# SuwoongHeo/neurecon

Hardware: AMD Instinct MI355X
Metric: rays/sec (4096 rays x 128 samples, 8-layer x256 SDF MLP) (higher is better)
Workload: dtype f16x3

## Files before the change

include/neurecon_hip.h:

```cpp
#ifndef NEURECON_HIP_H
#define NEURECON_HIP_H

#include <stddef.h>
#include <stdint.h>

#ifdef __cplusplus
extern "C" {
#endif

#define NR_OK 0
#define NR_ERR_ARG (-1)
#define NR_ERR_UNSUPPORTED (-2)
#define NR_ERR_HIP (-3)
#define NR_ERR_WORKSPACE (-4)

#define NR_PREC_FP32 0
#define NR_PREC_F16X3 1

#define NR_UPSAMPLE_OFFICIAL 0
#define NR_UPSAMPLE_DIRECT_USE 1
#define NR_UPSAMPLE_DIRECT_MORE 2

int nr_version(void);
const char* nr_last_error(void);
// ... 86 lines not shown
  float fixed_s;
  int N_nograd_samples;
  const float* t_nograd;
  void* workspace;
  size_t workspace_bytes;
  const float* u_rand;
  const float* t_out_rand;
  const float* s_dev;
  int sample_only;
  float* d_all_out;
  int no_mid_skip;
  int no_defer;
  int64_t max_chunk_rays;
  size_t max_workspace_bytes;
  const void* fold_packed;
} NrNeusArgs;

#define NR_DEFAULT_WORKSPACE_BYTES ((size_t)4 << 30)
#define NR_MIN_CHUNK_RAYS 4096

size_t nr_neus_workspace_bytes(const NrNeusArgs* a);
int nr_neus_render(const NrNeusArgs* a, void* stream);

size_t nr_neus_fold_packed_bytes(const NrSdfDesc* sdf, const NrRadDesc* rad);
int nr_neus_fold_pack(const NrSdfDesc* sdf, const NrRadDesc* rad, const float* W8, const float* b8, const float* W0,
                      const float* b0, void* packed, void* stream);
int nr_neus_fold_forward(const NrSdfDesc* sdf, const void* sdf_packed, const NrRadDesc* rad, const void* rad_packed,
                         const void* fold_packed, const float* pts, const float* vdir, int64_t vdir_div,
                         const float* normals, int64_t P, float* u, float* sdf_out, float* rgb, void* stream);

// ... 365 lines not shown
```

neurecon_amd/_lib.py:

```python
import ctypes
import os
import threading

import torch

HERE = os.path.dirname(os.path.abspath(__file__))
LIB_PATH = os.environ.get('NR_LIB', os.path.join(HERE, 'libnrhip.so'))

PREC_FP32 = 0
PREC_F16X3 = 1
UPSAMPLE = {'official_solution': 0, 'direct_use': 1, 'direct_more': 2}

_c_p = ctypes.c_void_p
_c_i = ctypes.c_int
_c_i64 = ctypes.c_int64
_c_f = ctypes.c_float
_c_d = ctypes.c_double
_c_sz = ctypes.c_size_t


class NrSdfDesc(ctypes.Structure):
    _fields_ = [('D', _c_i), ('W', _c_i), ('skip', _c_i), ('multires', _c_i), ('W_geo_feat', _c_i),
                ('precision', _c_i), ('siren', _c_i)]

# ... 14 lines not shown
        ('sdf', ctypes.POINTER(NrSdfDesc)), ('sdf_packed', _c_p),
        ('rad', ctypes.POINTER(NrRadDesc)), ('rad_packed', _c_p),
        ('s', _c_f), ('obj_bounding_radius', _c_f), ('near_bypass', _c_f), ('far_bypass', _c_f),
        ('N_samples', _c_i), ('N_importance', _c_i), ('N_upsample_iters', _c_i), ('calc_normal', _c_i),
        ('white_bkgd', _c_i),
        ('t_coarse', _c_p), ('u_fine', _c_p),
        ('rgb', _c_p), ('depth', _c_p), ('acc', _c_p), ('normals', _c_p),
        ('d_final', _c_p), ('sdf_out', _c_p), ('nablas_out', _c_p), ('radiance_out', _c_p),
        ('alpha_out', _c_p), ('cdf_out', _c_p), ('weights_out', _c_p),
        ('nerf', ctypes.POINTER(NrNerfDesc)), ('nerf_packed', _c_p), ('N_outside', _c_i), ('t_outside', _c_p),
        ('sigma_out', _c_p), ('radiance_bg_out', _c_p),
        ('upsample_algo', _c_i), ('fixed_s', _c_f), ('N_nograd_samples', _c_i), ('t_nograd', _c_p),
        ('workspace', _c_p), ('workspace_bytes', _c_sz),
        ('u_rand', _c_p), ('t_out_rand', _c_p), ('s_dev', _c_p), ('sample_only', _c_i), ('d_all_out', _c_p),
        ('no_mid_skip', _c_i), ('no_defer', _c_i), ('max_chunk_rays', _c_i64), ('max_workspace_bytes', _c_sz),
        ('fold_packed', _c_p),
    ]


class NrVolsdfArgs(ctypes.Structure):
    _fields_ = [
        ('rays_o', _c_p), ('rays_d', _c_p), ('n_rays', _c_i64),
        ('sdf', ctypes.POINTER(NrSdfDesc)), ('sdf_packed', _c_p),
        ('rad', ctypes.POINTER(NrRadDesc)), ('rad_packed', _c_p),
        ('alpha_net', _c_f), ('beta_net', _c_f), ('beta_plus_init', _c_f), ('eps', _c_f),
        ('near', _c_f), ('far', _c_f), ('obj_bounding_radius', _c_f), ('use_sphere_bg', _c_i),
        ('N_samples', _c_i), ('N_importance', _c_i), ('max_upsample_steps', _c_i), ('max_bisection_steps', _c_i),
        ('calc_normal', _c_i), ('white_bkgd', _c_i),
        ('t_coarse', _c_p), ('t_init', _c_p), ('u_up', _c_p), ('u_fine', _c_p),
        ('rgb', _c_p), ('depth', _c_p), ('acc', _c_p), ('normals', _c_p),
        ('d_vals', _c_p), ('sdf_out', _c_p), ('nablas_out', _c_p), ('radiance_out', _c_p),
# ... 287 lines not shown
```

neurecon_amd/csrc/nr_capi.hip:

```cpp
#include <algorithm>
#include <cmath>
#include <cstring>
#include <string>

#include "nr_common.h"
#include <cstdlib>
#include "nr_mlp.h"
#include "nr_tgemm.h"
#include "nr_neus.h"
#include "nr_volsdf.h"
#include "nr_unisurf.h"

namespace nr {

static thread_local std::string g_err;
void set_error(const std::string& msg) { g_err = msg; }

static size_t align256(size_t x) { return (x + 255) & ~(size_t)255; }
static int64_t chunk_bytes_host(int KB) { return (int64_t)(2 * KB + 1) * 1024; }

int check_sdf_desc(const NrSdfDesc* d) {
  NR_REQUIRE(d, NR_ERR_ARG, "null NrSdfDesc");
  if (d->siren) {
    NR_REQUIRE(d->D == 5 && d->W == 256 && d->skip < 0 && d->multires < 0 && d->W_geo_feat == 256,
// ... 183 lines not shown
  c.pts_nog = F(pl.o_ptsn); c.s_nog = F(pl.o_sn);
  const bool fused = !direct && !a.sample_only;
  c.nraw = fused ? c.nab_f : nullptr;
  c.idv = fused ? (int*)(ws + pl.o_idv) : nullptr;
  if (fused) {
    c.sdf_f = c.sv;
    c.nab_f = F(pl.o_nsort);
  }
  const bool defer = fused && neus_deferred(a, R);
  if (defer) {
    c.slabs = (float4*)(ws + pl.o_slabs);
    c.tflag = (int*)(ws + pl.o_tflag);
    c.tiles = (int*)(ws + pl.o_tiles);
    c.tcnt = (int*)(ws + pl.o_tcnt);
  }
  void* mlp_ws = ws + pl.o_mlp;
  const size_t mlp_bytes = a.workspace_bytes - pl.o_mlp;
  const SdfLayout SL = sdf_layout(*a.sdf);
  const RadLayout RL = rad_layout(*a.rad);
  auto sample_sdf = [&](const float* pts, int64_t P, float* sdf_out, int64_t slot0) -> int {
    if (defer)
      return launch_sdf_deferred(SL, a.sdf_packed, pts, P, sdf_out, nullptr, a.sdf->multires,
                                 (float4*)((char*)c.slabs + (size_t)(slot0 / 16) * kSlabColBytes), nullptr, nullptr,
                                 1, st);
    return launch_sdf(SL, a.sdf_packed, pts, P, sdf_out, fused ? c.nraw + slot0 * 3 : nullptr, nullptr,
                      a.sdf->multires, fused ? mlp_ws : nullptr, fused ? mlp_bytes : 0, st);
  };
  const dim3 blk(64), grd((R + 63) / 64);
  int rc;

  {
  ProfScope prof("neus_prologue", (double)R, st);
  hipLaunchKernelGGL(neus_prologue, grd, blk, 0, st, c, a.rays_o + ray0 * 3, a.rays_d + ray0 * 3, a.t_coarse,
                     a.obj_bounding_radius, a.near_bypass, a.far_bypass);
  }
  NR_HIP_CHECK(hipGetLastError());
  if (a.upsample_algo != NR_UPSAMPLE_DIRECT_MORE && (rc = sample_sdf(c.pts, (int64_t)a.N_samples * R, c.sv, 0)))
    return rc;
  if (a.upsample_algo == NR_UPSAMPLE_DIRECT_MORE) {
    hipLaunchKernelGGL(neus_nograd_points, grd, blk, 0, st, c);
    NR_HIP_CHECK(hipGetLastError());
    if ((rc = launch_sdf(SL, a.sdf_packed, c.pts_nog, (int64_t)c.n_nog * R, c.s_nog, nullptr, nullptr,
                         a.sdf->multires, nullptr, 0, st)))
      return rc;
  }
  if (direct) {
    ProfScope prof("neus_upsample", (double)R, st);
    const float* u = a.u_rand ? a.u_rand + ray0 * a.N_importance : a.u_fine;
    hipLaunchKernelGGL(neus_direct_upsample, grd, blk, 0, st, c, (int)(a.upsample_algo == NR_UPSAMPLE_DIRECT_MORE), u,
                       (int64_t)(a.u_rand ? a.N_importance : 0));
  }
  NR_HIP_CHECK(hipGetLastError());
  float* dvb[2] = {c.dv, F(pl.o_dv2)};
  float* svb[2] = {c.sv, F(pl.o_sv2)};
  int* idb[2] = {c.idv, fused ? (int*)(ws + pl.o_idv2) : nullptr};
  int cur = 0;
  auto merge = [&](int L) -> int {
    ProfScope prof("neus_merge", (double)R, st);
    const int64_t nt = (int64_t)(L + n_up) * R;
    hipLaunchKernelGGL(neus_merge, dim3((unsigned)((nt + 255) / 256)), dim3(256), 0, st, c, L, dvb[cur ^ 1],
                       svb[cur ^ 1], idb[cur ^ 1]);
    cur ^= 1;
    c.dv = dvb[cur];
    c.sv = svb[cur];
    c.idv = idb[cur];
    if (fused) c.sdf_f = c.sv;
    NR_HIP_CHECK(hipGetLastError());
    return NR_OK;
  };
  for (int it = 0; it < c.n_iters; ++it) {
    if (it > 0 && (rc = merge(a.N_samples + (it - 1) * n_up))) return rc;
    const int64_t slot0 = (int64_t)(a.N_samples + it * n_up) * R;
    NeusChunk cu = c;
    if (defer) cu.pts = c.pts + slot0 * 3;
    {
      ProfScope prof("neus_upsample", (double)R, st);
      const float* u = a.u_rand ? a.u_rand + ((int64_t)it * a.n_rays + ray0) * n_up : a.u_fine;
      const size_t lds1 = (5 * (size_t)c.S + 1) * sizeof(float);
      if (4 * lds1 <= 65536)
        hipLaunchKernelGGL((neus_upsample<4>), dim3((unsigned)((R + 3) / 4)), dim3(64), 4 * lds1, st, cu, it, u,
                           (int64_t)(a.u_rand ? n_up : 0));
      else
        hipLaunchKernelGGL((neus_upsample<1>), dim3((unsigned)R), dim3(64), lds1, st, cu, it, u,
                           (int64_t)(a.u_rand ? n_up : 0));
    }
    NR_HIP_CHECK(hipGetLastError());
    if ((rc = sample_sdf(cu.pts, (int64_t)n_up * R, c.snew, slot0))) return rc;
  }
  if (c.n_iters > 0 && (rc = merge(c.S - n_up))) return rc;
  if (defer) {
    const int64_t nslot = (int64_t)c.S * R;
    c.tshift = 0;
    NR_HIP_CHECK(hipMemsetAsync(c.nraw, 0, (size_t)nslot * 3 * sizeof(float), st));
    if (a.calc_normal && a.N_outside == 0) {
      NR_HIP_CHECK(hipMemsetAsync(c.tflag, 0, (size_t)nslot * sizeof(int), st));
      NR_HIP_CHECK(hipMemsetAsync(c.tcnt, 0, sizeof(int), st));
      const int64_t nq = (int64_t)(c.S - 1) * R;
      hipLaunchKernelGGL(neus_sample_need, dim3((unsigned)((nq + 255) / 256)), dim3(256), 0, st, c, a.s_dev, a.s);
      NR_HIP_CHECK(hipGetLastError());
      hipLaunchKernelGGL(neus_point_list, dim3((unsigned)((nslot + 1023) / 1024)), dim3(1024), 0, st, c, nslot);
      NR_HIP_CHECK(hipGetLastError());
      if ((rc = launch_sdf_deferred(SL, a.sdf_packed, c.pts, nslot, nullptr, c.nraw, a.sdf->multires, c.slabs, c.tiles,
                                    c.tcnt, 4, st)))
        return rc;
    }
  }
  if (a.sample_only) {
    hipLaunchKernelGGL(neus_write_dall, dim3((unsigned)(((int64_t)c.S * R + 255) / 256)), dim3(256), 0, st, c.dv,
                       (int64_t)R, c.S, ray0, a.d_all_out);
    NR_HIP_CHECK(hipGetLastError());
    return NR_OK;
  }
  {
    ProfScope prof("neus_points", (double)R, st);
    hipLaunchKernelGGL(neus_expand, dim3((unsigned)(((int64_t)c.S * R + 255) / 256)), dim3(256), 0, st, c,
                       (int)!(defer && a.N_outside > 0));
  }
  NR_HIP_CHECK(hipGetLastError());
  if (!fused && (rc = launch_sdf(SL, a.sdf_packed, c.pts, (int64_t)c.S * R, c.sdf_f, c.nab_f, nullptr,
                                 a.sdf->multires, mlp_ws, mlp_bytes, st)))
    return rc;
  const int64_t Pm = (int64_t)(c.S - 1) * R;
  const char* f8p = nullptr;
  const char* r0p = nullptr;
  if (a.fold_packed) {
    const FoldLayout FL = fold_layout(RL);
    f8p = (const char*)a.fold_packed + FL.f8_off;
    r0p = (const char*)a.fold_packed + FL.r0_off;
  }
  if (a.radiance_out || a.no_mid_skip) {
    if ((rc = launch_sdf(SL, a.sdf_packed, c.mids, Pm, c.sdf_m, c.nab_m, c.feat_m, a.sdf->multires, mlp_ws, mlp_bytes,
                         st, nullptr, 0, f8p)))
      return rc;
    if ((rc = launch_radiance(RL, a.rad_packed, c.mids, c.rd, 1, R, c.nab_m, c.feat_m, Pm, c.rad_m,
                              a.rad->multires_view, st, nullptr, r0p)))
      return rc;
  } else {
    char* wsb = (char*)a.workspace;
    int* cnt = (int*)(wsb + pl.o_mcnt);
    int* slot = (int*)(wsb + pl.o_mslot);
    float* midc = (float*)(wsb + pl.o_midc);
    float* vdc = (float*)(wsb + pl.o_mvd);
    float* radc = (float*)(wsb + pl.o_mrad);
    NR_HIP_CHECK(hipMemsetAsync(cnt, 0, sizeof(int), st));
    const dim3 g1((unsigned)((Pm + 255) / 256));
    hipLaunchKernelGGL(neus_mid_compact, dim3((unsigned)((Pm + 1023) / 1024)), dim3(1024), 0, st, c, a.s_dev, a.s, cnt,
                       slot, midc, vdc);
    NR_HIP_CHECK(hipGetLastError());
    if ((rc = launch_sdf(SL, a.sdf_packed, midc, Pm, c.sdf_m, c.nab_m, c.feat_m, a.sdf->multires, mlp_ws, mlp_bytes,
                         st, cnt, 1, f8p)))
      return rc;
    if ((rc = launch_radiance(RL, a.rad_packed, midc, vdc, 1, INT64_MAX, c.nab_m, c.feat_m, Pm, radc,
                              a.rad->multires_view, st, cnt, r0p)))
      return rc;
    hipLaunchKernelGGL(neus_mid_scatter, g1, dim3(256), 0, st, slot, radc, Pm, c.rad_m);
    NR_HIP_CHECK(hipGetLastError());
  }
  NeusOut o{ray0, a.rgb, a.depth, a.acc, a.normals, a.d_final, a.sdf_out, a.nablas_out,
            a.radiance_out, a.alpha_out, a.cdf_out, a.weights_out, a.sigma_out, a.radiance_bg_out};
  if (a.N_outside > 0) {
    hipLaunchKernelGGL(neus_outside_points, grd, blk, 0, st, c,
                       a.t_out_rand ? a.t_out_rand + ray0 * a.N_outside : (const float*)nullptr);
    NR_HIP_CHECK(hipGetLastError());
    const int64_t Po = (int64_t)(c.S - 1 + a.N_outside) * R;
    if (a.sigma_out || a.radiance_bg_out) {
      if ((rc = launch_nerf(nerf_layout(*a.nerf), a.nerf_packed, c.x4, c.rd, 1, R, Po, c.sig_o, c.rad_o, st)))
        return rc;
    } else {
      char* wsb = (char*)a.workspace;
      int* cnt = (int*)(wsb + pl.o_cnt);
      int* slot = (int*)(wsb + pl.o_slot);
// ... 4 lines not shown
      NR_HIP_CHECK(hipMemsetAsync(cnt, 0, sizeof(int), st));
      const dim3 g1((unsigned)((Po + 255) / 256));
      hipLaunchKernelGGL(neus_outside_compact, dim3((unsigned)((Po + 1023) / 1024)), dim3(1024), 0, st, c, cnt, slot,
                         x4c, vdc);
      NR_HIP_CHECK(hipGetLastError());
      if ((rc = launch_nerf(nerf_layout(*a.nerf), a.nerf_packed, x4c, vdc, 1, INT64_MAX, Po, sigc, radc, st, cnt)))
        return rc;
      hipLaunchKernelGGL(neus_outside_scatter, g1, dim3(256), 0, st, slot, sigc, radc, Po, c.sig_o, c.rad_o);
      NR_HIP_CHECK(hipGetLastError());
    }
    if (defer) {
      const int64_t nslot = (int64_t)c.S * R;
      c.tshift = 0;
      if (a.calc_normal) {
        NR_HIP_CHECK(hipMemsetAsync(c.tflag, 0, (size_t)nslot * sizeof(int), st));
        NR_HIP_CHECK(hipMemsetAsync(c.tcnt, 0, sizeof(int), st));
        hipLaunchKernelGGL(neus_sample_need_outside, dim3((unsigned)((nslot + 255) / 256)), dim3(256), 0, st, c,
                           a.s_dev, a.s);
        NR_HIP_CHECK(hipGetLastError());
        hipLaunchKernelGGL(neus_point_list, dim3((unsigned)((nslot + 1023) / 1024)), dim3(1024), 0, st, c, nslot);
        NR_HIP_CHECK(hipGetLastError());
        if ((rc = launch_sdf_deferred(SL, a.sdf_packed, c.pts, nslot, nullptr, c.nraw, a.sdf->multires, c.slabs,
                                      c.tiles, c.tcnt, 4, st)))
          return rc;
      }
      hipLaunchKernelGGL(neus_gather_nablas, dim3((unsigned)((nslot + 255) / 256)), dim3(256), 0, st, c);
      NR_HIP_CHECK(hipGetLastError());
    }
    ProfScope prof("neus_composite", (double)R, st);
    const int M = c.S - 1 + a.N_outside;
    const size_t lds1 = (6 * (size_t)M + 4 * (size_t)c.S) * sizeof(float);
// ... 904 lines not shown
```

neurecon_amd/csrc/nr_neus.h:

```cpp
#pragma once
#include "nr_common.h"

namespace nr {

constexpr int kMaxUp = 32;

struct NeusChunk {
  int R;
  int N_samples;
  int n_up;
  int n_iters;
  int S;
  float* ro; float* rd; float* near; float* far;
  float* dv; float* sv; float* wtmp; float* dnew; float* snew;
  float* pts; float* mids; float* dmid;
  float* sdf_f; float* nab_f;
  float* nraw; int* idv;
  float4* slabs; int* tflag; int* tiles; int* tcnt; int tshift;
  float* sdf_m; float* nab_m; float* feat_m; float* rad_m;
  int N_out;
  float r_obj;
  const float* t_out;
  float* d_out; float* x4; float* sig_o; float* rad_o;
  int n_imp;
  int n_nog;
  float fixed_s;
  const float* t_nog;
  float* pts_nog; float* s_nog;
};

struct NeusOut {
  int64_t ray0;
  float* rgb; float* depth; float* acc; float* normals;
// ... 10 lines not shown
  size_t o_mslot, o_midc, o_mvd, o_mrad, o_mcnt;
  size_t o_slabs, o_tflag, o_tiles, o_tcnt;
  size_t total;
};

NeusPlan neus_plan(const NrNeusArgs& a, int64_t Rc);
bool neus_deferred(const NrNeusArgs& a, int64_t R);
int neus_total_samples(const NrNeusArgs& a);
__global__ void neus_sample_need(NeusChunk c, const float* s_dev, float s_val);
__global__ void neus_tile_list(NeusChunk c, int64_t n_tiles);
__global__ void neus_point_list(NeusChunk c, int64_t n_slots);
__global__ void neus_sample_need_outside(NeusChunk c, const float* s_dev, float s_val);
__global__ void neus_gather_nablas(NeusChunk c);

__global__ void neus_prologue(NeusChunk c, const float* rays_o, const float* rays_d, const float* t_coarse,
                              float r_obj, float near_bypass, float far_bypass);
template <int RPW>
__global__ void neus_upsample(NeusChunk c, int it, const float* u, int64_t u_stride);
__global__ void neus_merge(NeusChunk c, int L, float* dv2, float* sv2, int* idv2);
__global__ void neus_expand(NeusChunk c, int gather);
template <int RPW>
__global__ void neus_composite(NeusChunk c, NeusOut o, const float* s_dev, float s_val, int calc_normal, int white_bkgd);
__global__ void neus_outside_points(NeusChunk c, const float* t_rand);
__global__ void neus_outside_compact(NeusChunk c, int* count, int* slot, float* x4c, float* vdc);
__global__ void neus_mid_compact(NeusChunk c, const float* s_dev, float s_val, int* count, int* slot, float* midc,
                                 float* vdc);
__global__ void neus_mid_scatter(const int* slot, const float* radc, int64_t n, float* rad_m);
__global__ void neus_outside_scatter(const int* slot, const float* sigc, const float* radc, int64_t n, float* sig_o,
                                     float* rad_o);
__global__ void neus_nograd_points(NeusChunk c);
__global__ void neus_direct_upsample(NeusChunk c, int more, const float* u, int64_t u_stride);
__global__ void neus_composite_outside(NeusChunk c, NeusOut o, const float* s_dev, float s_val, int calc_normal,
                                       int white_bkgd);
// ... 9 lines not shown
```

neurecon_amd/csrc/nr_neus.hip:

```cpp
#include "nr_common.h"
#include "nr_mlp.h"
#include "nr_neus.h"

namespace nr {

__device__ __forceinline__ float4 load3(const float* p) { return make_float4(p[0], p[1], p[2], 0.f); }

__device__ __forceinline__ void normalize3(float& x, float& y, float& z) {
  const float n = norm3_ref(x, y, z);
  const float d = fmaxf(n, 1e-12f);
  x = fdiv(x, d);
  y = fdiv(y, d);
  z = fdiv(z, d);
}

__global__ __launch_bounds__(64) void neus_prologue(NeusChunk c, const float* __restrict__ rays_o, const float* __restrict__ rays_d,
                              const float* __restrict__ t_coarse, float r_obj, float near_bypass, float far_bypass) {
  const int r = blockIdx.x * blockDim.x + threadIdx.x;
  if (r >= c.R) return;
  const float ox = rays_o[r * 3 + 0], oy = rays_o[r * 3 + 1], oz = rays_o[r * 3 + 2];
  float dx = rays_d[r * 3 + 0], dy = rays_d[r * 3 + 1], dz = rays_d[r * 3 + 2];
  normalize3(dx, dy, dz);
  c.ro[r * 3 + 0] = ox; c.ro[r * 3 + 1] = oy; c.ro[r * 3 + 2] = oz;
  c.rd[r * 3 + 0] = dx; c.rd[r * 3 + 1] = dy; c.rd[r * 3 + 2] = dz;
  const float mid = -fadd(fadd(fmul(ox, dx), fmul(oy, dy)), fmul(oz, dz));
  float nr = fmaxf(fsub(mid, r_obj), 0.0f);
  float fr = fmaxf(fadd(mid, r_obj), r_obj);
  if (!__builtin_isnan(near_bypass)) nr = near_bypass;
  if (!__builtin_isnan(far_bypass)) fr = far_bypass;
  c.near[r] = nr;
  c.far[r] = fr;
  for (int s = 0; s < c.N_samples; ++s) {
    const float t = t_coarse[s];
// ... 41 lines not shown
    w[i * stride] = (float)acc;
  }
  auto cdf = [&](int j) { return j == 0 ? 0.0f : w[(int64_t)(j - 1) * stride]; };
  for (int k = 0; k < n; ++k) {
    const float uk = u[k];
    int lo = 0, hi = L;
    while (lo < hi) {
      const int m = (lo + hi) >> 1;
      if (cdf(m) >= uk) hi = m; else lo = m + 1;
    }
    const int below = lo > 0 ? lo - 1 : 0, above = lo < L - 1 ? lo : L - 1;
    out[k * out_stride] = invert_one(uk, cdf(below), cdf(above), bins[below * stride], bins[above * stride]);
  }
}

template <int RPW>
__global__ __launch_bounds__(64) void neus_upsample(NeusChunk c, int it, const float* __restrict__ u, int64_t u_stride) {
  extern __shared__ float lds[];
  constexpr int NL = 64 / RPW;
  const int r = blockIdx.x * RPW + (int)threadIdx.x / NL, l = (int)threadIdx.x % NL;
  const int L = c.N_samples + it * c.n_up;
  const int64_t R = c.R;
  const bool live = r < R;
  const int Ll = live ? L : 0;
  float* sz = lds + ((int)threadIdx.x / NL) * (5 * c.S + 1);
  float* ss = sz + c.S;
  float* sa = ss + c.S;
  float* scdf = sa + c.S;
  float* sq = scdf + c.S;
  float* stot = sq + c.S;
  for (int i = l; i < Ll; i += NL) {
    sz[i] = c.dv[i * R + r];
    ss[i] = c.sv[i * R + r];
  }
  __syncthreads();
  const float S = (float)(64 << it);
  for (int i = l; i < Ll - 1; i += NL) {
    const float s0 = ss[i], s1 = ss[i + 1], z0 = sz[i], z1 = sz[i + 1];
    const float mid = fmul(fadd(s0, s1), 0.5f);
    const float slope = fdiv(fsub(s1, s0), fadd(fsub(z1, z0), 1e-5f));
    const float prev_slope = i > 0 ? fdiv(fsub(s0, ss[i - 1]), fadd(fsub(z0, sz[i - 1]), 1e-5f)) : 0.0f;
    float m = fminf(prev_slope, slope);
    m = fminf(fmaxf(m, -10.0f), 0.0f);
    const float dist = fsub(z1, z0);
    const float md = fmul(fmul(m, dist), 0.5f);
    const float c0 = sigmoidf_ref(fmul(fsub(mid, md), S));
    const float c1 = sigmoidf_ref(fmul(fadd(mid, md), S));
    const float alpha = fdiv(fadd(fsub(c0, c1), 1e-5f), fadd(c0, 1e-5f));
    sa[i] = alpha;
    scdf[i] = fadd(fsub(1.0f, alpha), 1e-10f);
// ... 33 lines not shown
    } else {
      int lo = 0, hi = L - 1;
      while (lo < hi) {
        const int mm = (lo + hi) >> 1;
        if (uk <= scdf[mm + 1]) hi = mm; else lo = mm + 1;
      }
      d = lo < L - 1 ? invert_one(uk, scdf[lo], scdf[lo + 1], sz[lo], sz[lo + 1])
                     : invert_one(uk, scdf[L - 1], scdf[L - 1], sz[L - 1], sz[L - 1]);
    }
    const int64_t q = k * R + r;
    c.dnew[q] = d;
    c.pts[q * 3 + 0] = fadd(ox, fmul(dx, d));
    c.pts[q * 3 + 1] = fadd(oy, fmul(dy, d));
    c.pts[q * 3 + 2] = fadd(oz, fmul(dz, d));
  }
}

template __global__ void neus_upsample<1>(NeusChunk, int, const float*, int64_t);
template __global__ void neus_upsample<4>(NeusChunk, int, const float*, int64_t);

__device__ __forceinline__ float merge_key(float v) { return v != v ? __builtin_inff() : v; }

__global__ void neus_merge(NeusChunk c, int L, float* __restrict__ dv2, float* __restrict__ sv2,
                           int* __restrict__ idv2) {
  const int64_t R = c.R;
  const int n = c.n_up;
  const int64_t t = (int64_t)blockIdx.x * blockDim.x + threadIdx.x;
  if (t >= (int64_t)(L + n) * R) return;
  const int64_t e = t / R, r = t - e * R;
  if (e < L) {
    const int64_t q = e * R + r;
    const float d = c.dv[q], kd = merge_key(d);
    int cnt = 0;
    for (int k = 0; k < n; ++k) cnt += merge_key(c.dnew[k * R + r]) < kd ? 1 : 0;
    const int64_t qo = (e + cnt) * R + r;
    dv2[qo] = d;
// ... 76 lines not shown
  float* snrm = srad + 3 * S;
  float* sdm = snrm + 3 * S;
  for (int i = l; i < Sl; i += NL) {
    const float cdf = sigmoidf_ref(fmul(c.sdf_f[i * R + r], s_inv));
    scdf[i] = cdf;
    if (o.cdf) o.cdf[ro * S + i] = cdf;
  }
  __syncthreads();
  for (int i = l; i < Sl - 1; i += NL) {
    const float cp = scdf[i], cn = scdf[i + 1];
    const float alpha = fmaxf(fdiv(fsub(cp, cn), fadd(cp, 1e-10f)), 0.0f);
    sal[i] = alpha;
    if (o.alpha) o.alpha[ro * (S - 1) + i] = alpha;
    const int64_t q = i * R + r;
    sdm[i] = c.dmid[q];
#pragma unroll
    for (int e = 0; e < 3; ++e) srad[i * 3 + e] = c.rad_m[q * 3 + e];
    if (calc_normal) {
      float x = c.nab_f[q * 3 + 0], y = c.nab_f[q * 3 + 1], z = c.nab_f[q * 3 + 2];
      normalize3(x, y, z);
      snrm[i * 3 + 0] = x;
      snrm[i * 3 + 1] = y;
      snrm[i * 3 + 2] = z;
    }
  }
  __syncthreads();
  double rgb0 = 0.0, rgb1 = 0.0, rgb2 = 0.0, n0 = 0.0, n1 = 0.0, n2 = 0.0;
  float accf = 0.0f;
  if (l == 0 && live) {
    double T = 1.0, acc = 0.0;
    for (int i = 0; i < S - 1; ++i) {
      const float alpha = sal[i];
      const float w = fmul(alpha, (float)T);
      T *= (double)fadd(fsub(1.0f, alpha), 1e-10f);
// ... 324 lines not shown

__global__ void neus_tile_list(NeusChunk c, int64_t n_tiles) {
  const int64_t t = (int64_t)blockIdx.x * blockDim.x + threadIdx.x;
  const bool need = t < n_tiles && c.tflag[t] != 0;
  const int64_t j = block_append(need, c.tcnt);
  if (need) c.tiles[j] = (int)t;
}

__global__ void neus_mid_scatter(const int* __restrict__ slot, const float* __restrict__ radc, int64_t n,
                                 float* __restrict__ rad_m) {
  const int64_t q = (int64_t)blockIdx.x * blockDim.x + threadIdx.x;
  if (q >= n) return;
  const int j = slot[q];
#pragma unroll
  for (int e = 0; e < 3; ++e) rad_m[q * 3 + e] = j < 0 ? 0.0f : radc[(int64_t)j * 3 + e];
}

__global__ void neus_outside_scatter(const int* __restrict__ slot, const float* __restrict__ sigc,
                                     const float* __restrict__ radc, int64_t n, float* __restrict__ sig_o,
                                     float* __restrict__ rad_o) {
  const int64_t q = (int64_t)blockIdx.x * blockDim.x + threadIdx.x;
  if (q >= n) return;
  const int j = slot[q];
  if (j < 0) return;
  sig_o[q] = sigc[j];
  rad_o[q * 3 + 0] = radc[(int64_t)j * 3 + 0];
  rad_o[q * 3 + 1] = radc[(int64_t)j * 3 + 1];
  rad_o[q * 3 + 2] = radc[(int64_t)j * 3 + 2];
}

// ... 339 lines not shown
```

neurecon_amd/frameworks/neus.py:

```python
import copy
import ctypes
import math
from collections import OrderedDict

import numpy as np
import torch
import torch.nn as nn
import torch.nn.functional as F

from .. import _lib as L
from ..base import ImplicitSurface, NeRF, RadianceNet, _no_training, check_view_dirs, wants_graph
from .. import rend_util


class NeuS(nn.Module):

    def __init__(self, variance_init=0.05, speed_factor=1.0, input_ch=3, W_geo_feat=-1, use_outside_nerf=False,
                 obj_bounding_radius=1.0, surface_cfg=dict(), radiance_cfg=dict()):
        super().__init__()
        self.ln_s = nn.Parameter(data=torch.Tensor([-np.log(variance_init) / speed_factor]), requires_grad=True)
        self.speed_factor = speed_factor
        self.implicit_surface = ImplicitSurface(W_geo_feat=W_geo_feat, input_ch=input_ch,
                                                obj_bounding_size=obj_bounding_radius, **surface_cfg)
        if W_geo_feat < 0:
# ... 41 lines not shown
            outs.append(rend_util.to_device(rend_util.uniform([*pre, nc, N_outside]).float(), dev))
    u = None
    if ups:
        u = torch.cat(ups, rd)
        u = (u.reshape(B * N, N_importance) if direct else u.reshape(n_iters, B * N, n_up)).contiguous()
    t_out = torch.cat(outs, len(pre)).reshape(B * N, N_outside).contiguous() if outs else None
    return u, t_out


def volume_render(rays_o, rays_d, model, obj_bounding_radius=1.0, batched=False, batched_info={},
                  calc_normal=False, use_view_dirs=True, rayschunk=65536, netchunk=1048576, white_bkgd=False,
                  near_bypass=None, far_bypass=None, detailed_output=True, show_progress=False, perturb=False,
                  fixed_s_recp=1 / 64., N_samples=64, N_importance=64, N_outside=0,
                  upsample_algo='official_solution', N_nograd_samples=2048, N_upsample_iters=4,
                  skip_zero_alpha=True, defer_sample_nablas=True, max_workspace_gb=None, fold_feature=True,
                  **dummy_kwargs):
    L.require_gpu(rays_o, 'rays_o')
    if wants_graph(model):
        return _train_render(rays_o, rays_d, model, obj_bounding_radius=obj_bounding_radius, batched=batched,
                             calc_normal=calc_normal, use_view_dirs=use_view_dirs, rayschunk=rayschunk,
                             white_bkgd=white_bkgd, near_bypass=near_bypass, far_bypass=far_bypass,
                             detailed_output=detailed_output, perturb=perturb, fixed_s_recp=fixed_s_recp,
                             N_samples=N_samples, N_importance=N_importance, N_outside=N_outside,
                             upsample_algo=upsample_algo, N_nograd_samples=N_nograd_samples,
                             N_upsample_iters=N_upsample_iters)
    if upsample_algo not in L.UPSAMPLE:
        raise NotImplementedError(upsample_algo)
    direct = upsample_algo != 'official_solution'
    check_view_dirs(model, use_view_dirs)
    dev = rays_o.device
    if batched:
# ... 28 lines not shown
                   radiance=torch.empty(n, M, 3, device=dev), alpha=torch.empty(n, M, device=dev),
                   cdf=torch.empty(n, S, device=dev), visibility_weights=torch.empty(n, M, device=dev),
                   d_final=torch.empty(n, M, device=dev))
        if N_outside > 0:
            det['sigma_out'] = torch.empty(n, M, device=dev)
            det['radiance_out'] = torch.empty(n, M, 3, device=dev)
    a = L.NrNeusArgs()
    a.rays_o, a.rays_d, a.n_rays = L.ptr(ro), L.ptr(rd), n
    a.sdf, a.sdf_packed = ctypes.pointer(sdf_desc), L.ptr(sdf_packed)
    a.rad, a.rad_packed = ctypes.pointer(rad_desc), L.ptr(rad_packed)
    fold_packed = model.radiance_net.nr_fold_packed(model.implicit_surface, dev) if fold_feature else None
    a.fold_packed = L.ptr(fold_packed)
    a.s, a.s_dev = 0.0, L.ptr(s_dev)
    a.no_mid_skip = 0 if skip_zero_alpha else 1
    a.no_defer = 0 if defer_sample_nablas else 1
    a.max_chunk_rays = int(rayschunk) if rayschunk else 0
    a.max_workspace_bytes = L.workspace_budget_bytes(max_workspace_gb)
    a.obj_bounding_radius = float(obj_bounding_radius)
    a.near_bypass = float('nan') if near_bypass is None else float(near_bypass)
    a.far_bypass = float('nan') if far_bypass is None else float(far_bypass)
    a.N_samples, a.N_importance, a.N_upsample_iters = N_samples, N_importance, N_upsample_iters
    a.calc_normal, a.white_bkgd = int(bool(calc_normal)), int(bool(white_bkgd))
    a.t_coarse, a.u_fine = L.ptr(t_coarse), L.ptr(u_fine)
    a.upsample_algo = L.UPSAMPLE[upsample_algo]
    a.fixed_s = 1. / fixed_s_recp
    if upsample_algo == 'direct_more':
        t_nograd = _linspace_table(N_nograd_samples, dev)
        a.N_nograd_samples, a.t_nograd = N_nograd_samples, L.ptr(t_nograd)
    a.rgb, a.depth, a.acc, a.normals = L.ptr(rgb), L.ptr(depth), L.ptr(acc), L.ptr(normals)
    a.d_final = L.ptr(det.get('d_final'))
# ... 30 lines not shown
        ret['implicit_nablas'] = det['implicit_nablas'].reshape(*prefix, S, 3)
        ret['implicit_surface'] = det['implicit_surface'].reshape(*prefix, S)
        ret['radiance'] = det['radiance'].reshape(*prefix, M, 3)
        ret['alpha'] = det['alpha'].reshape(*prefix, M)
        ret['cdf'] = det['cdf'].reshape(*prefix, S)
        ret['visibility_weights'] = det['visibility_weights'].reshape(*prefix, M)
        ret['d_final'] = det['d_final'].reshape(*prefix, M)
        if N_outside > 0:
            ret['sigma_out'] = det['sigma_out'].reshape(*prefix, M)
            ret['radiance_out'] = det['radiance_out'].reshape(*prefix, M, 3)
    return ret['rgb'], ret['depth_volume'], ret


def _sample_depths(ro, rd, model, dev, obj_bounding_radius, batched, B, rayschunk, near_bypass, far_bypass, perturb,
                   fixed_s_recp, N_samples, N_importance, upsample_algo, N_nograd_samples, N_upsample_iters,
                   N_outside=0):
    direct = upsample_algo != 'official_solution'
    n = ro.shape[0]
    n_up = N_importance if direct else (N_importance // N_upsample_iters if N_upsample_iters > 0 else 0)
    S = N_samples + (N_importance if direct else N_upsample_iters * n_up)
    sdf_desc, sdf_packed = model.implicit_surface.nr_packed(dev)
    rad_desc = model.radiance_net.nr_desc()
    d_all = torch.empty(n, S, device=dev)
    a = L.NrNeusArgs()
    a.rays_o, a.rays_d, a.n_rays = L.ptr(ro), L.ptr(rd), n
    a.sdf, a.sdf_packed = ctypes.pointer(sdf_desc), L.ptr(sdf_packed)
    a.rad, a.rad_packed = ctypes.pointer(rad_desc), None
    a.obj_bounding_radius = float(obj_bounding_radius)
    a.near_bypass = float('nan') if near_bypass is None else float(near_bypass)
    a.far_bypass = float('nan') if far_bypass is None else float(far_bypass)
    a.N_samples, a.N_importance, a.N_upsample_iters = N_samples, N_importance, N_upsample_iters
    t_coarse = _linspace_table(N_samples, dev)
    u_fine = _linspace_table(max(n_up, 1), dev)
    a.t_coarse, a.u_fine = L.ptr(t_coarse), L.ptr(u_fine)
    a.upsample_algo = L.UPSAMPLE[upsample_algo]
    a.fixed_s = 1. / fixed_s_recp
    if upsample_algo == 'direct_more':
        t_nograd = _linspace_table(N_nograd_samples, dev)
        a.N_nograd_samples, a.t_nograd = N_nograd_samples, L.ptr(t_nograd)
    t_out = None
    if perturb:
        u_rand, t_out = _neus_uniforms(B, n // B, batched, int(rayschunk), direct, N_upsample_iters, n_up,
                                       N_importance, N_outside, dev)
        a.u_rand = L.ptr(u_rand)
    a.sample_only, a.d_all_out = 1, L.ptr(d_all)
    a.max_chunk_rays = int(rayschunk) if rayschunk else 0
    a.max_workspace_bytes = L.workspace_budget_bytes()
    lib = L.lib()
    ws_bytes = lib.nr_neus_workspace_bytes(ctypes.byref(a))
    ws = L.workspace(dev, ws_bytes)
    a.workspace, a.workspace_bytes = L.ptr(ws), ws_bytes
    L.check(lib.nr_neus_render(ctypes.byref(a), L.stream_of(dev)))
    return d_all, t_out


def _outside_depths(ro, rd, obj_bounding_radius, far_bypass, N_outside, t_out):
    _, far = rend_util.near_far_from_sphere(ro, rd, r=obj_bounding_radius)
    if far_bypass is not None:
        far = far_bypass * torch.ones_like(far)
    t = torch.linspace(0, 1, N_outside + 2)[..., 1:-1].float().to(ro.device)
# ... 201 lines not shown
```

Baseline: 695,100.

## Fuse merge into upsample and finalize, compact mid-samples inside finalize kernel

The per-iteration merge kernel is folded into the next upsample kernel's LDS staging. The final merge, tflag computation, dmid computation and mid-point compaction are folded into a new neus_finalize kernel. Atomic counters are now zeroed in the prologue instead of by separate memsets, and the mid scatter is dropped by having the compositing kernel read the compact radiance through slot indices. The aim is to cut kernel launches, memsets and global round trips, at the cost of more LDS use and more complex kernels.

```diff
diff --git a/include/neurecon_hip.h b/include/neurecon_hip.h
--- a/include/neurecon_hip.h
+++ b/include/neurecon_hip.h
@@ -124,6 +124,7 @@
   int64_t max_chunk_rays;
   size_t max_workspace_bytes;
   const void* fold_packed;
+  int no_chain_fuse;
 } NrNeusArgs;
 
 #define NR_DEFAULT_WORKSPACE_BYTES ((size_t)4 << 30)
diff --git a/neurecon_amd/_lib.py b/neurecon_amd/_lib.py
--- a/neurecon_amd/_lib.py
+++ b/neurecon_amd/_lib.py
@@ -52,7 +52,7 @@
         ('workspace', _c_p), ('workspace_bytes', _c_sz),
         ('u_rand', _c_p), ('t_out_rand', _c_p), ('s_dev', _c_p), ('sample_only', _c_i), ('d_all_out', _c_p),
         ('no_mid_skip', _c_i), ('no_defer', _c_i), ('max_chunk_rays', _c_i64), ('max_workspace_bytes', _c_sz),
-        ('fold_packed', _c_p),
+        ('fold_packed', _c_p), ('no_chain_fuse', _c_i),
     ]
 
 
diff --git a/neurecon_amd/csrc/nr_capi.hip b/neurecon_amd/csrc/nr_capi.hip
--- a/neurecon_amd/csrc/nr_capi.hip
+++ b/neurecon_amd/csrc/nr_capi.hip
@@ -221,6 +221,11 @@
     c.tiles = (int*)(ws + pl.o_tiles);
     c.tcnt = (int*)(ws + pl.o_tcnt);
   }
+  const bool chain = !a.no_chain_fuse;
+  const bool mid_skip = !a.sample_only && !(a.radiance_out || a.no_mid_skip);
+  const size_t fin_lds = (size_t)kFinRays * 6 * c.S * sizeof(float);
+  const bool chain_fin = chain && defer && a.N_outside == 0 && mid_skip && fin_lds <= 65536;
+  int* const mcnt = (int*)(ws + pl.o_mcnt);
   void* mlp_ws = ws + pl.o_mlp;
   const size_t mlp_bytes = a.workspace_bytes - pl.o_mlp;
   const SdfLayout SL = sdf_layout(*a.sdf);
@@ -239,7 +244,8 @@
   {
   ProfScope prof("neus_prologue", (double)R, st);
   hipLaunchKernelGGL(neus_prologue, grd, blk, 0, st, c, a.rays_o + ray0 * 3, a.rays_d + ray0 * 3, a.t_coarse,
-                     a.obj_bounding_radius, a.near_bypass, a.far_bypass);
+                     a.obj_bounding_radius, a.near_bypass, a.far_bypass, chain && defer ? c.tcnt : (int*)nullptr,
+                     chain && mid_skip ? mcnt : (int*)nullptr);
   }
   NR_HIP_CHECK(hipGetLastError());
   if (a.upsample_algo != NR_UPSAMPLE_DIRECT_MORE && (rc = sample_sdf(c.pts, (int64_t)a.N_samples * R, c.sv, 0)))
@@ -262,46 +268,78 @@
   float* svb[2] = {c.sv, F(pl.o_sv2)};
   int* idb[2] = {c.idv, fused ? (int*)(ws + pl.o_idv2) : nullptr};
   int cur = 0;
+  auto flip = [&]() {
+    cur ^= 1;
+    c.dv = dvb[cur];
+    c.sv = svb[cur];
+    c.idv = idb[cur];
+    if (fused) c.sdf_f = c.sv;
+  };
   auto merge = [&](int L) -> int {
     ProfScope prof("neus_merge", (double)R, st);
     const int64_t nt = (int64_t)(L + n_up) * R;
     hipLaunchKernelGGL(neus_merge, dim3((unsigned)((nt + 255) / 256)), dim3(256), 0, st, c, L, dvb[cur ^ 1],
                        svb[cur ^ 1], idb[cur ^ 1]);
-    cur ^= 1;
-    c.dv = dvb[cur];
-    c.sv = svb[cur];
-    c.idv = idb[cur];
-    if (fused) c.sdf_f = c.sv;
+    flip();
     NR_HIP_CHECK(hipGetLastError());
     return NR_OK;
   };
   for (int it = 0; it < c.n_iters; ++it) {
-    if (it > 0 && (rc = merge(a.N_samples + (it - 1) * n_up))) return rc;
+    const bool merge_here = chain && it > 0;
+    if (it > 0 && !chain && (rc = merge(a.N_samples + (it - 1) * n_up))) return rc;
     const int64_t slot0 = (int64_t)(a.N_samples + it * n_up) * R;
     NeusChunk cu = c;
     if (defer) cu.pts = c.pts + slot0 * 3;
     {
       ProfScope prof("neus_upsample", (double)R, st);
       const float* u = a.u_rand ? a.u_rand + ((int64_t)it * a.n_rays + ray0) * n_up : a.u_fine;
-      const size_t lds1 = (5 * (size_t)c.S + 1) * sizeof(float);
+      const size_t lds1 = (5 * (size_t)c.S + 1 + (merge_here ? c.S : 0)) * sizeof(float);
+      float* const mg_d = merge_here ? dvb[cur ^ 1] : nullptr;
+      float* const mg_s = merge_here ? svb[cur ^ 1] : nullptr;
+      int* const mg_i = merge_here ? idb[cur ^ 1] : nullptr;
       if (4 * lds1 <= 65536)
         hipLaunchKernelGGL((neus_upsample<4>), dim3((unsigned)((R + 3) / 4)), dim3(64), 4 * lds1, st, cu, it, u,
-                           (int64_t)(a.u_rand ? n_up : 0));
+                           (int64_t)(a.u_rand ? n_up : 0), mg_d, mg_s, mg_i);
       else
         hipLaunchKernelGGL((neus_upsample<1>), dim3((unsigned)R), dim3(64), lds1, st, cu, it, u,
-                           (int64_t)(a.u_rand ? n_up : 0));
+                           (int64_t)(a.u_rand ? n_up : 0), mg_d, mg_s, mg_i);
     }
     NR_HIP_CHECK(hipGetLastError());
+    if (merge_here) flip();
     if ((rc = sample_sdf(cu.pts, (int64_t)n_up * R, c.snew, slot0))) return rc;
   }
-  if (c.n_iters > 0 && (rc = merge(c.S - n_up))) return rc;
-  if (defer) {
+  int* const mslot = (int*)(ws + pl.o_mslot);
+  float* const midc = F(pl.o_midc);
+  float* const mvd = F(pl.o_mvd);
+  float* const mrad = F(pl.o_mrad);
+  if (chain_fin) {
+    const int64_t nslot = (int64_t)c.S * R;
+    c.tshift = 0;
+    {
+      ProfScope prof("neus_points", (double)R, st);
+      hipLaunchKernelGGL(neus_finalize, dim3((unsigned)((R + kFinRays - 1) / kFinRays)), dim3(256), fin_lds, st, c,
+                         c.n_iters > 0 ? n_up : 0, dvb[cur ^ 1], svb[cur ^ 1], idb[cur ^ 1], a.s_dev, a.s, a.calc_normal,
+                         mcnt, mslot, midc, mvd);
+    }
+    NR_HIP_CHECK(hipGetLastError());
+    flip();
+    if (a.calc_normal) {
+      hipLaunchKernelGGL(neus_point_list, dim3((unsigned)((nslot + 1023) / 1024)), dim3(1024), 0, st, c, nslot);
+      NR_HIP_CHECK(hipGetLastError());
+      if ((rc = launch_sdf_deferred(SL, a.sdf_packed, c.pts, nslot, nullptr, c.nraw, a.sdf->multires, c.slabs, c.tiles,
+                                    c.tcnt, 4, st)))
+        return rc;
+    }
+  } else if (c.n_iters > 0 && (rc = merge(c.S - n_up))) {
+    return rc;
+  }
+  if (defer && !chain_fin) {
     const int64_t nslot = (int64_t)c.S * R;
     c.tshift = 0;
     NR_HIP_CHECK(hipMemsetAsync(c.nraw, 0, (size_t)nslot * 3 * sizeof(float), st));
     if (a.calc_normal && a.N_outside == 0) {
       NR_HIP_CHECK(hipMemsetAsync(c.tflag, 0, (size_t)nslot * sizeof(int), st));
-      NR_HIP_CHECK(hipMemsetAsync(c.tcnt, 0, sizeof(int), st));
+      if (!chain) NR_HIP_CHECK(hipMemsetAsync(c.tcnt, 0, sizeof(int), st));
       const int64_t nq = (int64_t)(c.S - 1) * R;
       hipLaunchKernelGGL(neus_sample_need, dim3((unsigned)((nq + 255) / 256)), dim3(256), 0, st, c, a.s_dev, a.s);
       NR_HIP_CHECK(hipGetLastError());
@@ -318,7 +356,7 @@
     NR_HIP_CHECK(hipGetLastError());
     return NR_OK;
   }
-  {
+  if (!chain_fin) {
     ProfScope prof("neus_points", (double)R, st);
     hipLaunchKernelGGL(neus_expand, dim3((unsigned)(((int64_t)c.S * R + 255) / 256)), dim3(256), 0, st, c,
                        (int)!(defer && a.N_outside > 0));
@@ -343,25 +381,26 @@
                               a.rad->multires_view, st, nullptr, r0p)))
       return rc;
   } else {
-    char* wsb = (char*)a.workspace;
-    int* cnt = (int*)(wsb + pl.o_mcnt);
-    int* slot = (int*)(wsb + pl.o_mslot);
-    float* midc = (float*)(wsb + pl.o_midc);
-    float* vdc = (float*)(wsb + pl.o_mvd);
-    float* radc = (float*)(wsb + pl.o_mrad);
-    NR_HIP_CHECK(hipMemsetAsync(cnt, 0, sizeof(int), st));
-    const dim3 g1((unsigned)((Pm + 255) / 256));
-    hipLaunchKernelGGL(neus_mid_compact, dim3((unsigned)((Pm + 1023) / 1024)), dim3(1024), 0, st, c, a.s_dev, a.s, cnt,
-                       slot, midc, vdc);
-    NR_HIP_CHECK(hipGetLastError());
+    if (!chain_fin) {
+      if (!chain) NR_HIP_CHECK(hipMemsetAsync(mcnt, 0, sizeof(int), st));
+      hipLaunchKernelGGL(neus_mid_compact, dim3((unsigned)((Pm + 1023) / 1024)), dim3(1024), 0, st, c, a.s_dev, a.s,
+                         mcnt, mslot, midc, mvd);
+      NR_HIP_CHECK(hipGetLastError());
+    }
     if ((rc = launch_sdf(SL, a.sdf_packed, midc, Pm, c.sdf_m, c.nab_m, c.feat_m, a.sdf->multires, mlp_ws, mlp_bytes,
-                         st, cnt, 1, f8p)))
+                         st, mcnt, 1, f8p)))
       return rc;
-    if ((rc = launch_radiance(RL, a.rad_packed, midc, vdc, 1, INT64_MAX, c.nab_m, c.feat_m, Pm, radc,
-                              a.rad->multires_view, st, cnt, r0p)))
+    if ((rc = launch_radiance(RL, a.rad_packed, midc, mvd, 1, INT64_MAX, c.nab_m, c.feat_m, Pm, mrad,
+                              a.rad->multires_view, st, mcnt, r0p)))
       return rc;
-    hipLaunchKernelGGL(neus_mid_scatter, g1, dim3(256), 0, st, slot, radc, Pm, c.rad_m);
-    NR_HIP_CHECK(hipGetLastError());
+    if (chain_fin) {
+      c.cslot = mslot;
+      c.cradc = mrad;
+    } else {
+      hipLaunchKernelGGL(neus_mid_scatter, dim3((unsigned)((Pm + 255) / 256)), dim3(256), 0, st, mslot, mrad, Pm,
+                         c.rad_m);
+      NR_HIP_CHECK(hipGetLastError());
+    }
   }
   NeusOut o{ray0, a.rgb, a.depth, a.acc, a.normals, a.d_final, a.sdf_out, a.nablas_out,
             a.radiance_out, a.alpha_out, a.cdf_out, a.weights_out, a.sigma_out, a.radiance_bg_out};
@@ -396,7 +435,7 @@
       c.tshift = 0;
       if (a.calc_normal) {
         NR_HIP_CHECK(hipMemsetAsync(c.tflag, 0, (size_t)nslot * sizeof(int), st));
-        NR_HIP_CHECK(hipMemsetAsync(c.tcnt, 0, sizeof(int), st));
+        if (!chain) NR_HIP_CHECK(hipMemsetAsync(c.tcnt, 0, sizeof(int), st));
         hipLaunchKernelGGL(neus_sample_need_outside, dim3((unsigned)((nslot + 255) / 256)), dim3(256), 0, st, c,
                            a.s_dev, a.s);
         NR_HIP_CHECK(hipGetLastError());
diff --git a/neurecon_amd/csrc/nr_neus.h b/neurecon_amd/csrc/nr_neus.h
--- a/neurecon_amd/csrc/nr_neus.h
+++ b/neurecon_amd/csrc/nr_neus.h
@@ -4,6 +4,7 @@
 namespace nr {
 
 constexpr int kMaxUp = 32;
+constexpr int kFinRays = 16;
 
 struct NeusChunk {
   int R;
@@ -17,6 +18,7 @@
   float* sdf_f; float* nab_f;
   float* nraw; int* idv;
   float4* slabs; int* tflag; int* tiles; int* tcnt; int tshift;
+  const int* cslot; const float* cradc;
   float* sdf_m; float* nab_m; float* feat_m; float* rad_m;
   int N_out;
   float r_obj;
@@ -57,9 +59,12 @@
 __global__ void neus_gather_nablas(NeusChunk c);
 
 __global__ void neus_prologue(NeusChunk c, const float* rays_o, const float* rays_d, const float* t_coarse,
-                              float r_obj, float near_bypass, float far_bypass);
+                              float r_obj, float near_bypass, float far_bypass, int* zero0, int* zero1);
 template <int RPW>
-__global__ void neus_upsample(NeusChunk c, int it, const float* u, int64_t u_stride);
+__global__ void neus_upsample(NeusChunk c, int it, const float* u, int64_t u_stride, float* dv2, float* sv2,
+                              int* idv2);
+__global__ void neus_finalize(NeusChunk c, int n_new, float* dv2, float* sv2, int* idv2, const float* s_dev,
+                              float s_val, int flags, int* count, int* slot, float* midc, float* vdc);
 __global__ void neus_merge(NeusChunk c, int L, float* dv2, float* sv2, int* idv2);
 __global__ void neus_expand(NeusChunk c, int gather);
 template <int RPW>
diff --git a/neurecon_amd/csrc/nr_neus.hip b/neurecon_amd/csrc/nr_neus.hip
--- a/neurecon_amd/csrc/nr_neus.hip
+++ b/neurecon_amd/csrc/nr_neus.hip
@@ -15,8 +15,13 @@
 }
 
 __global__ __launch_bounds__(64) void neus_prologue(NeusChunk c, const float* __restrict__ rays_o, const float* __restrict__ rays_d,
-                              const float* __restrict__ t_coarse, float r_obj, float near_bypass, float far_bypass) {
+                              const float* __restrict__ t_coarse, float r_obj, float near_bypass, float far_bypass,
+                              int* __restrict__ zero0, int* __restrict__ zero1) {
   const int r = blockIdx.x * blockDim.x + threadIdx.x;
+  if (r == 0) {
+    if (zero0) *zero0 = 0;
+    if (zero1) *zero1 = 0;
+  }
   if (r >= c.R) return;
   const float ox = rays_o[r * 3 + 0], oy = rays_o[r * 3 + 1], oz = rays_o[r * 3 + 2];
   float dx = rays_d[r * 3 + 0], dy = rays_d[r * 3 + 1], dz = rays_d[r * 3 + 2];
@@ -88,8 +93,57 @@
   }
 }
 
+__device__ __forceinline__ float merge_key(float v) { return v != v ? __builtin_inff() : v; }
+
+template <int NL, int LS>
+__device__ __forceinline__ void merge_stage(const NeusChunk& c, int64_t r, int l, int Lo, int n, float* stage,
+                                            float* tS, int* tI, float* dD, float* dS, int* dI) {
+  const int64_t R = c.R;
+  for (int i = l; i < Lo; i += NL) {
+    const int64_t q = i * R + r;
+    stage[i * LS] = c.dv[q];
+    tS[i * LS] = c.sv[q];
+    if (dI) tI[i * LS] = c.idv[q];
+  }
+  for (int j = l; j < n; j += NL) {
+    stage[(Lo + j) * LS] = c.dnew[j * R + r];
+    tS[(Lo + j) * LS] = c.snew[j * R + r];
+  }
+  __syncthreads();
+  float nk[kMaxUp];
+#pragma unroll
+  for (int k = 0; k < kMaxUp; ++k) nk[k] = k < n ? merge_key(stage[(Lo + k) * LS]) : __builtin_inff();
+  for (int i = l; i < Lo; i += NL) {
+    const float d = stage[i * LS], kd = merge_key(d);
+    int cnt = 0;
+#pragma unroll
+    for (int k = 0; k < kMaxUp; ++k) cnt += nk[k] < kd ? 1 : 0;
+    const int pos = i + cnt;
+    dD[pos * LS] = d;
+    dS[pos * LS] = tS[i * LS];
+    if (dI) dI[pos * LS] = tI[i * LS];
+  }
+  for (int j = l; j < n; j += NL) {
+    const float d = stage[(Lo + j) * LS], kd = merge_key(d);
+    int rank = 0;
+#pragma unroll
+    for (int k = 0; k < kMaxUp; ++k) rank += (nk[k] < kd || (nk[k] == kd && k < j)) ? 1 : 0;
+    int lo = 0, hi = Lo;
+    while (lo < hi) {
+      const int m = (lo + hi) >> 1;
+      if (merge_key(stage[m * LS]) <= kd) lo = m + 1; else hi = m;
+    }
+    const int pos = rank + lo;
+    dD[pos * LS] = d;
+    dS[pos * LS] = tS[(Lo + j) * LS];
+    if (dI) dI[pos * LS] = Lo + j;
+  }
+  __syncthreads();
+}
+
 template <int RPW>
-__global__ __launch_bounds__(64) void neus_upsample(NeusChunk c, int it, const float* __restrict__ u, int64_t u_stride) {
+__global__ __launch_bounds__(64) void neus_upsample(NeusChunk c, int it, const float* __restrict__ u, int64_t u_stride,
+                                                    float* dv2, float* sv2, int* idv2) {
   extern __shared__ float lds[];
   constexpr int NL = 64 / RPW;
   const int r = blockIdx.x * RPW + (int)threadIdx.x / NL, l = (int)threadIdx.x % NL;
@@ -103,11 +157,17 @@
   float* scdf = sa + c.S;
   float* sq = scdf + c.S;
   float* stot = sq + c.S;
-  for (int i = l; i < Ll; i += NL) {
-    sz[i] = c.dv[i * R + r];
-    ss[i] = c.sv[i * R + r];
-  }
-  __syncthreads();
+  int* const sid = (int*)(lds + RPW * (5 * c.S + 1)) + ((int)threadIdx.x / NL) * c.S;
+  if (dv2) {
+    merge_stage<NL, 1>(c, r, l, live ? L - c.n_up : 0, live ? c.n_up : 0, scdf, sa, (int*)sq, sz, ss,
+                       idv2 ? sid : (int*)nullptr);
+  } else {
+    for (int i = l; i < Ll; i += NL) {
+      sz[i] = c.dv[i * R + r];
+      ss[i] = c.sv[i * R + r];
+    }
+    __syncthreads();
+  }
   const float S = (float)(64 << it);
   for (int i = l; i < Ll - 1; i += NL) {
     const float s0 = ss[i], s1 = ss[i + 1], z0 = sz[i], z1 = sz[i + 1];
@@ -171,12 +231,18 @@
     c.pts[q * 3 + 1] = fadd(oy, fmul(dy, d));
     c.pts[q * 3 + 2] = fadd(oz, fmul(dz, d));
   }
-}
-
-template __global__ void neus_upsample<1>(NeusChunk, int, const float*, int64_t);
-template __global__ void neus_upsample<4>(NeusChunk, int, const float*, int64_t);
-
-__device__ __forceinline__ float merge_key(float v) { return v != v ? __builtin_inff() : v; }
+  if (dv2) {
+    for (int i = l; i < L; i += NL) {
+      const int64_t q = i * R + r;
+      dv2[q] = sz[i];
+      sv2[q] = ss[i];
+      if (idv2) idv2[q] = sid[i];
+    }
+  }
+}
+
+template __global__ void neus_upsample<1>(NeusChunk, int, const float*, int64_t, float*, float*, int*);
+template __global__ void neus_upsample<4>(NeusChunk, int, const float*, int64_t, float*, float*, int*);
 
 __global__ void neus_merge(NeusChunk c, int L, float* __restrict__ dv2, float* __restrict__ sv2,
                            int* __restrict__ idv2) {
@@ -283,10 +349,22 @@
     if (o.alpha) o.alpha[ro * (S - 1) + i] = alpha;
     const int64_t q = i * R + r;
     sdm[i] = c.dmid[q];
+    float x = 0.0f, y = 0.0f, z = 0.0f;
+    if (c.cslot) {
+      const int j = c.cslot[q];
+      const int64_t qs = (int64_t)c.idv[q] * R + r, jj = j < 0 ? 0 : j;
+      const float v0 = c.cradc[jj * 3 + 0], v1 = c.cradc[jj * 3 + 1], v2 = c.cradc[jj * 3 + 2];
+      if (calc_normal) x = c.nraw[qs * 3 + 0], y = c.nraw[qs * 3 + 1], z = c.nraw[qs * 3 + 2];
+      srad[i * 3 + 0] = j < 0 ? 0.0f : v0;
+      srad[i * 3 + 1] = j < 0 ? 0.0f : v1;
+      srad[i * 3 + 2] = j < 0 ? 0.0f : v2;
+      if (alpha == 0.0f) x = 0.0f, y = 0.0f, z = 0.0f;
+    } else {
 #pragma unroll
-    for (int e = 0; e < 3; ++e) srad[i * 3 + e] = c.rad_m[q * 3 + e];
+      for (int e = 0; e < 3; ++e) srad[i * 3 + e] = c.rad_m[q * 3 + e];
+      if (calc_normal) x = c.nab_f[q * 3 + 0], y = c.nab_f[q * 3 + 1], z = c.nab_f[q * 3 + 2];
+    }
     if (calc_normal) {
-      float x = c.nab_f[q * 3 + 0], y = c.nab_f[q * 3 + 1], z = c.nab_f[q * 3 + 2];
       normalize3(x, y, z);
       snrm[i * 3 + 0] = x;
       snrm[i * 3 + 1] = y;
@@ -641,6 +719,86 @@
   const int j = slot[q];
 #pragma unroll
   for (int e = 0; e < 3; ++e) rad_m[q * 3 + e] = j < 0 ? 0.0f : radc[(int64_t)j * 3 + e];
+}
+
+__global__ __launch_bounds__(256) void neus_finalize(NeusChunk c, int n_new, float* __restrict__ dv2,
+                                                     float* __restrict__ sv2, int* __restrict__ idv2,
+                                                     const float* __restrict__ s_dev, float s_val, int flags,
+                                                     int* __restrict__ count, int* __restrict__ slot,
+                                                     float* __restrict__ midc, float* __restrict__ vdc) {
+  extern __shared__ float lds[];
+  __shared__ int wtot[4];
+  __shared__ int bbase;
+  constexpr int NL = 16, LS = kFinRays;
+  const int g = (int)threadIdx.x % LS, l = (int)threadIdx.x / LS;
+  const int S = c.S;
+  const int64_t R = c.R, r = (int64_t)blockIdx.x * LS + g;
+  const bool live = r < R;
+  const int Sl = live ? S : 0;
+  float* sz = lds + g;
+  float* ss = sz + LS * S;
+  int* si = (int*)(ss + LS * S);
+  float* st = ss + 2 * LS * S;
+  merge_stage<NL, LS>(c, r, l, live ? S - n_new : 0, live ? n_new : 0, st, st + LS * S, (int*)(st + 2 * LS * S), sz, ss,
+                      si);
+  const float s_inv = s_dev ? *s_dev : s_val;
+  uint32_t mask = 0;
+  {
+    int k = 0;
+    for (int i = l; i < Sl - 1; i += NL, ++k) {
+      const int64_t q = i * R + r;
+      const float cp = sigmoidf_ref(fmul(ss[i * LS], s_inv));
+      const float cn = sigmoidf_ref(fmul(ss[(i + 1) * LS], s_inv));
+      const float alpha = fmaxf(fdiv(fsub(cp, cn), fadd(cp, 1e-10f)), 0.0f);
+      const bool need = !(alpha == 0.0f);
+      c.dmid[q] = fmul(0.5f, fadd(sz[(i + 1) * LS], sz[i * LS]));
+      if (flags) c.tflag[(int64_t)si[i * LS] * R + r] = need ? 1 : 0;
+      if (need) mask |= 1u << k;
+    }
+    if (flags && live && l == 0) c.tflag[(int64_t)si[(S - 1) * LS] * R + r] = 0;
+  }
+  for (int i = l; i < Sl; i += NL) {
+    const int64_t q = i * R + r;
+    dv2[q] = sz[i * LS];
+    sv2[q] = ss[i * LS];
+    idv2[q] = si[i * LS];
+  }
+  const int mine = __popc(mask), lane = (int)threadIdx.x & 63, w = (int)threadIdx.x >> 6;
+  int incl = mine;
+#pragma unroll
+  for (int d = 1; d < 64; d <<= 1) {
+    const int v = __shfl_up(incl, d);
+    if (lane >= d) incl += v;
+  }
+  if (lane == 63) wtot[w] = incl;
+  __syncthreads();
+  if (threadIdx.x == 0) {
+    const int tot = wtot[0] + wtot[1] + wtot[2] + wtot[3];
+    bbase = tot ? atomicAdd(count, tot) : 0;
+  }
+  __syncthreads();
+  if (!live) return;
+  int64_t j = (int64_t)bbase + incl - mine;
+  for (int ww = 0; ww < w; ++ww) j += wtot[ww];
+  const float ox = c.ro[r * 3], oy = c.ro[r * 3 + 1], oz = c.ro[r * 3 + 2];
+  const float dx = c.rd[r * 3], dy = c.rd[r * 3 + 1], dz = c.rd[r * 3 + 2];
+  int k = 0;
+  for (int i = l; i < S - 1; i += NL, ++k) {
+    const int64_t q = i * R + r;
+    if ((mask >> k) & 1u) {
+      const float dm = fmul(0.5f, fadd(sz[(i + 1) * LS], sz[i * LS]));
+      slot[q] = (int)j;
+      midc[j * 3 + 0] = fadd(ox, fmul(dx, dm));
+      midc[j * 3 + 1] = fadd(oy, fmul(dy, dm));
+      midc[j * 3 + 2] = fadd(oz, fmul(dz, dm));
+      vdc[j * 3 + 0] = dx;
+      vdc[j * 3 + 1] = dy;
+      vdc[j * 3 + 2] = dz;
+      ++j;
+    } else {
+      slot[q] = -1;
+    }
+  }
 }
 
 __global__ void neus_outside_scatter(const int* __restrict__ slot, const float* __restrict__ sigc,
diff --git a/neurecon_amd/frameworks/neus.py b/neurecon_amd/frameworks/neus.py
--- a/neurecon_amd/frameworks/neus.py
+++ b/neurecon_amd/frameworks/neus.py
@@ -79,7 +79,7 @@
                   fixed_s_recp=1 / 64., N_samples=64, N_importance=64, N_outside=0,
                   upsample_algo='official_solution', N_nograd_samples=2048, N_upsample_iters=4,
                   skip_zero_alpha=True, defer_sample_nablas=True, max_workspace_gb=None, fold_feature=True,
-                  **dummy_kwargs):
+                  fuse_chain=True, **dummy_kwargs):
     L.require_gpu(rays_o, 'rays_o')
     if wants_graph(model):
         return _train_render(rays_o, rays_d, model, obj_bounding_radius=obj_bounding_radius, batched=batched,
@@ -138,6 +138,7 @@
     a.s, a.s_dev = 0.0, L.ptr(s_dev)
     a.no_mid_skip = 0 if skip_zero_alpha else 1
     a.no_defer = 0 if defer_sample_nablas else 1
+    a.no_chain_fuse = 0 if fuse_chain else 1
     a.max_chunk_rays = int(rayschunk) if rayschunk else 0
     a.max_workspace_bytes = L.workspace_budget_bytes(max_workspace_gb)
     a.obj_bounding_radius = float(obj_bounding_radius)
@@ -198,7 +199,7 @@
 
 def _sample_depths(ro, rd, model, dev, obj_bounding_radius, batched, B, rayschunk, near_bypass, far_bypass, perturb,
                    fixed_s_recp, N_samples, N_importance, upsample_algo, N_nograd_samples, N_upsample_iters,
-                   N_outside=0):
+                   N_outside=0, fuse_chain=True):
     direct = upsample_algo != 'official_solution'
     n = ro.shape[0]
     n_up = N_importance if direct else (N_importance // N_upsample_iters if N_upsample_iters > 0 else 0)
@@ -228,6 +229,7 @@
                                        N_importance, N_outside, dev)
         a.u_rand = L.ptr(u_rand)
     a.sample_only, a.d_all_out = 1, L.ptr(d_all)
+    a.no_chain_fuse = 0 if fuse_chain else 1
     a.max_chunk_rays = int(rayschunk) if rayschunk else 0
     a.max_workspace_bytes = L.workspace_budget_bytes()
     lib = L.lib()
```

Measured after the change: 695,000 (median of 2 runs). No clear change (-0.0%).
